# rnissel/Channel-Estimation

Measured on AMD Instinct MI355X. Metric: Monte-Carlo channel realisations/sec at 24sc x 14sym; BER curve match vs ref, higher is better.
Workload: dtype f64; 1 GPU; C2: OFDM 24sc x 14sym, N=540, Jakes 500 km/h VehA, 256-QAM, 16 pilots, 7 SNR (10:5:40 dB) x (one-tap + 4 IC) x (MMSE + perfect CSI); engine_batch=65536, parallelism=dp1

## Files before the change

channel-estimation_amd/csrc/dsce_api.hip:

```cpp
#include <math.h>
#include <stdlib.h>
#include <string.h>

#include <algorithm>
#include <functional>
#include <map>
#include <memory>
#include <stdexcept>
#include <string>
#include <cstdio>
#include <thread>
#include <vector>

#include <rccl/rccl.h>
#include <rocprofiler-sdk-roctx/roctx.h>

#include "dsce.h"
#include "dsce_kernels.h"

struct TraceRange {
    explicit TraceRange(const char* m) { roctxRangePushA(m); }
    ~TraceRange() { roctxRangePop(); }
    TraceRange(const TraceRange&) = delete;
    TraceRange& operator=(const TraceRange&) = delete;
// ... 1662 lines not shown
        if (r2 != DSCE_OK) return api_fail(ctx, r2, member_name(ctx, m) + ": " + member(ctx, m)->err);
    }
    return DSCE_OK;
}

template <class F>
static int fanout_par(dsce_ctx* ctx, F&& f) {
    if (!ctx || ctx->peers.empty()) return f(ctx);
    const size_t n = ctx->peers.size() + 1;
    std::vector<int> rc(n, DSCE_OK);
    std::vector<std::thread> th;
    try {
        for (size_t m = 1; m < n; ++m) th.emplace_back([&, m] { rc[m] = f(member(ctx, m)); });
    } catch (const std::exception& e) {
        for (auto& t : th) t.join();
        return api_fail(ctx, DSCE_ENOMEM, std::string("cannot start a member thread: ") + e.what());
    }
    rc[0] = f(ctx);
    for (auto& t : th) t.join();
    if (rc[0] != DSCE_OK) return rc[0];
    for (size_t m = 1; m < n; ++m)
        if (rc[m] != DSCE_OK) return api_fail(ctx, rc[m], member_name(ctx, m) + ": " + member(ctx, m)->err);
    return DSCE_OK;
}

static void shard_slice(uint64_t first, uint64_t n, size_t world, size_t m, uint64_t& f, uint64_t& k) {
    const uint64_t blocks = (n + 63) / 64;
    const uint64_t lo = std::min<uint64_t>(blocks * m / world * 64, n);
    const uint64_t hi = std::min<uint64_t>(blocks * (m + 1) / world * 64, n);
    f = first + lo;
    k = hi - lo;
}

extern "C" {

int dsce_abi_version(void) { return DSCE_ABI_VERSION; }

int dsce_device_count(int* count) {
    int n = 0;
    if (hipGetDeviceCount(&n) != hipSuccess) n = 0;
    if (count) *count = n;
    return DSCE_OK;
}

int dsce_create(int hip_device, dsce_ctx** out) {
    if (!out) return DSCE_EINVAL;
    *out = nullptr;
    auto* ctx = new (std::nothrow) dsce_ctx();
    if (!ctx) return DSCE_ENOMEM;
    ctx->device = hip_device;
    try {
        DSCE_HIP_CHECK(hipSetDevice(hip_device));
        DSCE_HIP_CHECK(hipStreamCreateWithFlags(&ctx->stream, hipStreamNonBlocking));
    } catch (const std::exception& e) {
        delete ctx;
        return DSCE_EHIP;
    }
    *out = ctx;
    return DSCE_OK;
}

int dsce_create_multi(const int32_t* devices, int32_t n_devices, dsce_ctx** out) {
    if (!out) return DSCE_EINVAL;
    *out = nullptr;
    if (!devices || n_devices < 1 || n_devices > 64) {
        fprintf(stderr, "dsce_create_multi: 1..64 devices expected\n");
        return DSCE_EINVAL;
    }
    int count = 0;
    if (hipGetDeviceCount(&count) != hipSuccess) count = 0;
    bool distinct = true;
    for (int i = 0; i < n_devices; ++i) {
        if (devices[i] < 0 || devices[i] >= count) {
            fprintf(stderr, "dsce_create_multi: device %d of %d is not a HIP device\n", (int)devices[i], count);
            return DSCE_EINVAL;
        }
        for (int j = 0; j < i; ++j) distinct = distinct && devices[j] != devices[i];
    }
    dsce_ctx* ctx = nullptr;
    int rc = dsce_create(devices[0], &ctx);
    if (rc != DSCE_OK) return rc;
    for (int i = 1; i < n_devices; ++i) {
        dsce_ctx* p = nullptr;
        rc = dsce_create(devices[i], &p);
        if (rc != DSCE_OK) {
            (void)dsce_destroy(ctx);
            return rc;
        }
        ctx->peers.push_back(p);
    }
    if (distinct) {
        ctx->comms.assign(n_devices, nullptr);
        const ncclResult_t r = ncclCommInitAll(ctx->comms.data(), n_devices, devices);
        if (r != ncclSuccess) {
            fprintf(stderr, "dsce_create_multi: ncclCommInitAll failed: %s\n", ncclGetErrorString(r));
            ctx->comms.clear();
            (void)dsce_destroy(ctx);
            return DSCE_EHIP;
        }
        ctx->reduce = DSCE_REDUCE_RCCL;
    } else {
        ctx->reduce = DSCE_REDUCE_HOST;
    }
    (void)hipSetDevice(devices[0]);
    *out = ctx;
    return DSCE_OK;
// ... 1059 lines not shown
            b += w.bytes;
        }
    }
    if (flops_per_rep) *flops_per_rep = f;
    if (bytes_per_rep) *bytes_per_rep = b;
    API_END
}

int dsce_structured_check(dsce_ctx* ctx, int32_t id, double* out) {
    API_BEGIN
    check_ctx(ctx);
    Scheme& s = get_scheme(ctx, id);
    if (!out) throw ApiError(DSCE_EINVAL, "null output");
    out[0] = s.mic_check;
    out[1] = s.mic_dev;
    out[2] = s.mic_wmax;
    out[3] = s.mic_rtol;
    out[4] = s.lr_resid;
    out[5] = s.Bz ? 1.0 : 0.0;
    out[6] = s.lr_ratio;
    API_END
}

int dsce_fp64_mfma_peak(dsce_ctx* ctx, double* tflops) {
    API_BEGIN
    check_ctx(ctx);
    if (!tflops) throw ApiError(DSCE_EINVAL, "null output");
    int cus = 0;
    DSCE_HIP_CHECK(hipDeviceGetAttribute(&cus, hipDeviceAttributeMultiprocessorCount, ctx->device));
    const int blocks = cus * 8, iters = 4096;
    double* out = dalloc<double>(ctx, (size_t)blocks * 256);
    hipEvent_t e0 = get_event(ctx), e1 = get_event(ctx);
    launch_mfma_f64_peak(ctx->stream, blocks, iters, out);
    float best = 1e30f;
    for (int rep = 0; rep < 3; ++rep) {
        DSCE_HIP_CHECK(hipEventRecord(e0, ctx->stream));
        launch_mfma_f64_peak(ctx->stream, blocks, iters, out);
        DSCE_HIP_CHECK(hipEventRecord(e1, ctx->stream));
        DSCE_HIP_CHECK(hipEventSynchronize(e1));
        float ms = 0.f;
        DSCE_HIP_CHECK(hipEventElapsedTime(&ms, e0, e1));
        best = ms < best ? ms : best;
    }
    DSCE_HIP_CHECK(hipGetLastError());
    ctx->event_pool.push_back(e0);
    ctx->event_pool.push_back(e1);
    free_alloc(ctx, out);
    *tflops = (double)blocks * 4 * iters * PEAK_MFMA_PER_ITER * 2048.0 / (best * 1e-3) / 1e12;
    API_END
}

#define DSCE_OPTIONS(X)                                                                                  \
    X(xcd) X(fuse_stage) X(pic_chain) X(pfuse) X(stage_split) X(noise_fuse) \
    X(snr_chunk) X(jakes_rpw) X(wtrim) X(wcontract_valu) X(mmse_ic) X(jakes_win) X(txrx_fft) X(snr_base) X(jakes_mom) X(realise_win) X(tx_rows) X(mic_lr) X(pic_poly) X(jakes_grp2) X(export_stage_mb)

static int set_option_one(dsce_ctx* ctx, const char* name, int64_t value) {
    API_BEGIN
    check_ctx(ctx);
    if (!name) throw ApiError(DSCE_EINVAL, "null option name");
    const std::string n(name);
    int* slot = nullptr;
#define X(f) if (n == #f) slot = &ctx->op.f;
    DSCE_OPTIONS(X)
#undef X
    if (!slot && (n == "pic_skip" || n == "ic_streams"))
        throw ApiError(DSCE_EINVAL, "option '" + n + "' was retired in r06 (measured neutral in r04 / r05; DESIGN.md 2.0d, 2.0f)");
    if (!slot && (n == "pic_net" || n == "mic_net" || n == "stage_rb" || n == "wrow"))
        throw ApiError(DSCE_EINVAL, "option '" + n + "' was retired: no scheme or channel selected its other values "
                                    "(DESIGN.md 2.0, Pruned after r06)");
    if (!slot) throw ApiError(DSCE_EINVAL, "unknown option '" + n + "'");
    if (n == "jakes_rpw" && value != 1 && value != 2) throw ApiError(DSCE_EINVAL, "jakes_rpw: 1 | 2");
    if (n == "pic_chain" && value != 0 && value != 3)
        throw ApiError(DSCE_EINVAL, "pic_chain: 0 (per-iteration passes) | 3 (k_pic_fft); the r01 chains 1 / 2 "
                                    "(k_pic_chain, k_pic_mfma) were retired in r03");
    if (n == "snr_base" && (value < 0 || value > 255)) throw ApiError(DSCE_EINVAL, "snr_base: 0..255");
    if (n == "snr_base") check_noise_streams(ctx, value, ctx->nsnr, max_noise_slot(ctx));
    if (n == "export_stage_mb" && value < 1) throw ApiError(DSCE_EINVAL, "export_stage_mb: >= 1 (MiB)");
    if (value < -1 || value > 1 << 20) throw ApiError(DSCE_EINVAL, "option value out of range");
    *slot = (int)value;
    API_END
}

int dsce_set_option(dsce_ctx* ctx, const char* name, int64_t value) {
    return fanout(ctx, [&](dsce_ctx* c) { return set_option_one(c, name, value); });
}

int dsce_get_option(dsce_ctx* ctx, const char* name, int64_t* value) {
    API_BEGIN
    if (!ctx || !name || !value) throw ApiError(DSCE_EINVAL, "null argument");
    const std::string n(name);
    const int* slot = nullptr;
#define X(f) if (n == #f) slot = &ctx->op.f;
    DSCE_OPTIONS(X)
#undef X
    if (!slot) throw ApiError(DSCE_EINVAL, "unknown option '" + n + "'");
    *value = *slot;
    API_END
}
#undef DSCE_OPTIONS

int dsce_path_info(dsce_ctx* ctx, int32_t id, uint32_t* flags) {
    API_BEGIN
    check_ctx(ctx);
    Scheme& s = get_scheme(ctx, id);
    if (!flags) throw ApiError(DSCE_EINVAL, "null output");
    *flags = s.path;
    API_END
}

int dsce_jakes_info(dsce_ctx* ctx, int32_t* out6) {
    API_BEGIN
    check_ctx(ctx);
    if (!out6) throw ApiError(DSCE_EINVAL, "null output");
    const JakesInfo& ji = ctx->jakes_info;
    out6[0] = ji.kernel;
    out6[1] = ji.grp2;
    out6[2] = ji.ngrp;
    out6[3] = ji.lg;
    out6[4] = ji.mt;
    out6[5] = ji.nchunk;
    API_END
}

int dsce_scheme_dims(dsce_ctx* ctx, int32_t id, dsce_dims* dims) {
    API_BEGIN
    if (!ctx) throw ApiError(DSCE_EINVAL, "null context");
    Scheme& s = get_scheme(ctx, id);
    if (!dims) throw ApiError(DSCE_EINVAL, "null output");
    dims->n_samples = s.N;
// ... 14 lines not shown
```

channel-estimation_amd/csrc/dsce_kernels.h:

```cpp
#pragma once

#include "dsce_common.h"

#include <vector>

namespace dsce {

struct Opts {
    int xcd = 1;
    int fuse_stage = 1;
    int pic_chain = 3;
    int pfuse = 1;
    int stage_split = 0;
    int noise_fuse = 1;
    int snr_chunk = 0;
    int jakes_rpw = 2;
    int wtrim = 1;
    int wcontract_valu = 0;
    int mmse_ic = 1;
    int jakes_win = 1;
    int txrx_fft = 1;
    int snr_base = 0;
    int tx_rows = 1;
    int realise_win = 0;
    int mic_lr = 1;
    int pic_poly = 1;
    int jakes_grp2 = 1;
    int jakes_mom = 2;
    int export_stage_mb = 1024;
};

enum : unsigned {
    PATH_WPAIR3_FUSED = 1u << 0,
    PATH_WPAIR3 = 1u << 1,
    PATH_WPAIR4M = 1u << 2,
    PATH_WCONTRACT_VALU = 1u << 3,
    PATH_PIC_MFMA = 1u << 4,
    PATH_PIC_CHAIN = 1u << 5,
    PATH_PIC_PASSES = 1u << 6,
    PATH_STAGE_FUSED = 1u << 7,
    PATH_STAGE_SPLIT = 1u << 8,
    PATH_NOISE_FUSED = 1u << 9,
    PATH_PIC_FFT = 1u << 10,
    PATH_MIC_FFT = 1u << 11,
    PATH_TXRX_FFT = 1u << 12,
    PATH_PILOT_FUSED = 1u << 13,
    PATH_MIC_STAGES = 1u << 14,
    PATH_MIC_LR = 1u << 15,
    PATH_PIC_POLY = 1u << 16,
    PATH_WROW3 = 1u << 17,
};

struct TraceK {
    int unit;
    int LK, ND;
    double2* yest;
    double2* yperf;
    double2* hest;
    int* dec_e;
    int* dec_p;
    int U;
};
__device__ __forceinline__ bool trace_hit(const TraceK* t, int unit) { return t->U > 0 || unit == t->unit; }
__device__ __forceinline__ size_t trace_ix(const TraceK* t, size_t e, int unit) {
    return t->U > 0 ? e * (size_t)t->U + (size_t)unit : e;
}
template <bool BULK>
__device__ __forceinline__ bool trace_hit(const TraceK* t, int unit) {
    if constexpr (BULK) return true;
    else return unit == t->unit;
}
template <bool BULK>
__device__ __forceinline__ size_t trace_ix(const TraceK* t, size_t e, int unit) {
    if constexpr (BULK) return e * (size_t)t->U + (size_t)unit;
    else return e;
}

struct McBuffers {
    int R;
    int rvalid;
    int nsnr;
    int U;
    int snr0;
    double2* ir;
    double2* xp;
    uint16_t* sidx;
    double2* r0;
    double2* h;
    double2* xs;
    double2* ss;
    double2* y;
    double2* yest;
    double2* yperf;
    double2* hp;
    double2* hp2;
    double2* hest;
    double2* v;
    double2* u;
    double2* t;
    double2* e;
    double2* e2;
    uint16_t* qe;
    uint16_t* qp;
// ... 162 lines not shown
```

channel-estimation_amd/csrc/kernels_mc.hip:

```cpp
#include "dsce_kernels.h"
#include "bm_tables.h"

#include <math.h>
#include <algorithm>
#include <stdexcept>
#include <type_traits>
#include <stdlib.h>
#include <string.h>

namespace dsce {

static constexpr double TWO_PI = 6.283185307179586;
static constexpr int WAVE = 64;

__device__ __forceinline__ int wave_sum(int v) {
#pragma unroll
    for (int o = 32; o > 0; o >>= 1) v += __shfl_xor(v, o, 64);
    return v;
}
__device__ __forceinline__ int wave_sum_dpp(int v) {
    v += __builtin_amdgcn_update_dpp(0, v, 0xb1, 0xf, 0xf, false);
    v += __builtin_amdgcn_update_dpp(0, v, 0x4e, 0xf, 0xf, false);
    v += __builtin_amdgcn_update_dpp(0, v, 0x141, 0xf, 0xf, false);
    v += __builtin_amdgcn_update_dpp(0, v, 0x140, 0xf, 0xf, false);
// ... 1401 lines not shown
    {0.25881904510252076, 0.96592582628906829},
    {0.0, 1.0},
    {-0.25881904510252076, 0.96592582628906829},
    {-0.5, 0.86602540378443865},
    {-0.70710678118654752, 0.70710678118654752},
    {-0.86602540378443865, 0.5},
    {-0.96592582628906829, 0.25881904510252076}};

template <int S>
__device__ __forceinline__ void dft3(double2& a, double2& b, double2& c) {
    constexpr double H = 0.86602540378443865;
    const double2 t = c_add(b, c), d = c_sub(b, c);
    const double2 m = make_double2(fma(-0.5, t.x, a.x), fma(-0.5, t.y, a.y));
    a = c_add(a, t);
    b = make_double2(fma(-S * H, d.y, m.x), fma(S * H, d.x, m.y));
    c = make_double2(fma(S * H, d.y, m.x), fma(-S * H, d.x, m.y));
}

__device__ __forceinline__ double2 c_mulf(double2 a, double2 b) {
    return make_double2(fma(a.x, b.x, -(a.y * b.y)), fma(a.x, b.y, a.y * b.x));
}


__device__ __forceinline__ double2 mfma4_cmul(double2 a, double2 b) {
    double re = __builtin_amdgcn_mfma_f64_4x4x4f64(a.x, b.x, 0.0, 0, 0, 0);
    re = __builtin_amdgcn_mfma_f64_4x4x4f64(a.y, b.y, re, 0, 0, 1);
    double im = __builtin_amdgcn_mfma_f64_4x4x4f64(a.x, b.y, 0.0, 0, 0, 0);
    im = __builtin_amdgcn_mfma_f64_4x4x4f64(a.y, b.x, im, 0, 0, 0);
    return make_double2(re, im);
}

__device__ __forceinline__ double2 bperm_c(int addr, double2 v) {
    return make_double2(__hiloint2double(__builtin_amdgcn_ds_bpermute(addr, __double2hiint(v.x)),
                                         __builtin_amdgcn_ds_bpermute(addr, __double2loint(v.x))),
                        __hiloint2double(__builtin_amdgcn_ds_bpermute(addr, __double2hiint(v.y)),
                                         __builtin_amdgcn_ds_bpermute(addr, __double2loint(v.y))));
}

__host__ __device__ constexpr int p6(int k) { return (6 - k) % 6; }

template <int S>
__device__ __forceinline__ void dft6(double2 (&x)[6]) {
    dft3<S>(x[0], x[2], x[4]);
    dft3<S>(x[3], x[5], x[1]);
#pragma unroll
    for (int k2 = 0; k2 < 3; ++k2) {
        const int i0 = 2 * k2, i1 = (2 * k2 + 3) % 6;
        const double2 a = x[i0], b = x[i1];
        x[i0] = c_add(a, b);
        x[i1] = c_sub(a, b);
    }
}

template <int NT, int SH, bool TRACE, bool S0>
__device__ __forceinline__ void pic_fft_body(const SchemeK& sk, const BandOrder& ord, const double2* __restrict__ ir, int N,
                                             const StorePerfectDetect& o, int niter, int vb, int vn) {
    int ug, blk;
    band_block(ord, sk.QH.nblk, ug, blk, vb, vn);
    const int tid = threadIdx.x, l = tid & 63, w = tid >> 6, r = l >> 4;
    const int U = o.U, R = o.R;
    const int unit = ug * WAVE + w * 16 + (l & 15);
    const int rl = unit % R;
    const int row0 = sk.QH.row0[blk], klo = sk.QH.klo[blk];
    const double cs = o.scI, rq = o.rQ;
    __shared__ double2 sym[256];
    __shared__ unsigned sgridw[64];
    const unsigned char* sgrid = (const unsigned char*)sgridw;
    __shared__ double2 rpv[24];
    __shared__ int rdc[24];
    __shared__ double2 amt[2][6][16];
    __shared__ int cntl[4][PM_MAXIT + 1];
    __shared__ double2 ucst[6][256];
    double2 u[6], yh[6], hc[6];
    unsigned txp[2] = {0u, 0u};
    double2 taps[6][NT];
    const __amdgpu_buffer_rsrc_t trs =
        buf_rsrc(ir + (size_t)klo * R, ((size_t)(NT - 1) * N + (N - klo)) * R * sizeof(double2));
    const unsigned tv0 = (unsigned)(6 * r * R + rl) * 16u;
    {
        const double2 a = sk.ct_symc[tid];
        const unsigned gw = sk.ct_grid[min(tid, 63)];
        const int rt = min(tid, 23);
        const double2 pv = sk.ct_rpv[blk * 24 + rt];
        const int rdv = sk.ct_rdc[blk * 24 + rt];
        const double2 nt = sk.ct_amt[min(tid, 191)];
        const RowView vu = S0 ? RowView(o.xs, row0, R, r, rl, 16) : RowView(o.u, row0, U, r, unit, 16);
        const RowView vs(o.sidr, row0, R, r, rl, 2), vy(o.y, row0, U, r, unit, 16), vh(o.h, row0, R, r, rl, 16);
#pragma unroll
        for (int b = 0; b < 6; ++b) {
            u[b] = vu.ld2(b);
            txp[b >> 2] |= (vs.ldu16(b) & 0xffu) << (8 * (b & 3));
            yh[b] = vy.ld2(b);
            hc[b] = vh.ld2(b);
        }
#pragma unroll
        for (int m = 0; m < 6; ++m)
#pragma unroll
            for (int q = 0; q < NT; ++q) taps[m][q] = buf_ld2(trs, tv0, (unsigned)((q * N + m) * R) * 16u);
        sym[tid] = a;
        sgridw[min(tid, 63)] = gw;
        rpv[rt] = pv;
        rdc[rt] = rdv;
        (&amt[0][0][0])[min(tid, 191)] = nt;
    }
    __syncthreads();
#pragma unroll
    for (int q = 0; q < NT; ++q) {
        double2 sq = taps[0][q];
#pragma unroll
        for (int m = 1; m < 6; ++m) sq = c_add(sq, taps[m][q]);
        sq = make_double2(__builtin_amdgcn_mfma_f64_4x4x4f64(1.0, sq.x, 0.0, 0, 0, 0),
                          __builtin_amdgcn_mfma_f64_4x4x4f64(1.0, sq.y, 0.0, 0, 0, 0));
        const double2 mq = make_double2(sq.x * (1.0 / 24.0), sq.y * (1.0 / 24.0));
#pragma unroll
        for (int m = 0; m < 6; ++m) taps[m][q] = c_sub(taps[m][q], mq);
    }
#pragma unroll
    for (int a = 0; a < 6; ++a) {
        u[a] = make_double2(u[a].x * cs, u[a].y * cs);
        ucst[a][tid] = u[a];
    }
    unsigned dmask = 0u, emask = 0u;
#pragma unroll
    for (int a = 0; a < 6; ++a) {
        const int dc = rdc[4 * a + r];
        dmask |= dc >= 0 ? 1u << a : 0u;
        emask |= dc >= 0 && (dc & 1) ? 1u << a : 0u;
    }
    int ncnt = 0;
    auto cweight = [&](int a) -> int {
        return ((dmask >> a) & 1) ? (((emask >> a) & 1) ? 0x10001 : 1) : 0;
    };
    auto reprecode = [&](const int (&dp)[6]) {
        double2 nv[6];
        if (o.pv_uni) {
#pragma unroll
            for (int a = 0; a < 6; ++a) nv[a] = ((dmask >> a) & 1) ? sym[dp[a]] : ucst[a][tid];
        } else {
#pragma unroll
            for (int a = 0; a < 6; ++a) {
                const double2 pr = c_mulf(rpv[4 * a + r], sym[dp[a]]), cv = ucst[a][tid];
                nv[a] = ((dmask >> a) & 1) ? pr : cv;
            }
        }
#pragma unroll
        for (int a = 0; a < 6; ++a) u[a] = nv[a];
    };
    if (S0) {
        int dp[6];
        double fI[6], fQ[6];
#pragma unroll
        for (int a = 0; a < 6; ++a) {
            const double2 hh = hc[a], yv = yh[a];
            const double id = recip_fast(hh.x * hh.x + hh.y * hh.y);
            hc[a] = make_double2(hh.x * id, -hh.y * id);
            const double2 ys = c_mulf(yv, hc[a]);
            yh[a] = make_double2(fma(ys.x, cs, o.ofI), ys.y * cs);
            fI[a] = yh[a].x;
            fQ[a] = fma(yh[a].y, rq, o.ofQ);
        }
        slice6(dp, fI, fQ, o.topI, o.topQ, sgrid);
#pragma unroll
        for (int a = 0; a < 6; ++a) {
            const bool data = (dmask >> a) & 1;
            ncnt += __umul24(__popc((unsigned)(dp[a] ^ (int)((txp[a >> 2] >> (8 * (a & 3))) & 0xffu))), cweight(a));
            if (TRACE && data && trace_hit(o.tr, unit)) o.tr->dec_p[trace_ix(o.tr, (size_t)(rdc[4 * a + r] >> 1), unit)] = dp[a];
        }
        reprecode(dp);
        cntl[w][0] = wave_sum_dpp(rl < o.rvalid ? ncnt : 0);
        ncnt = 0;
    }
    for (int it = 1; it <= niter; ++it) {
        int oz = 0;
        asm volatile("" : "+v"(oz));
        double2 x[6];
#pragma unroll
        for (int a = 0; a < 6; ++a) x[a] = u[a];
        dft6<1>(x);
        double2 t[6];
        const int ai = (l & 3) + 4 * (l >> 4) + oz;
#pragma unroll
        for (int m = 0; m < 6; ++m) {
            const double2 am = amt[0][m][ai], b = x[p6(m)];
            t[m] = mfma4_cmul(am, b);
        }
        const double2 tprev = bperm_c(((l + 48) & 63) * 4, t[5]);
#pragma unroll
        for (int m = 5; m >= 0; --m) {
            const double2 tp = m ? t[m - 1] : tprev;
            double2 acc = make_double2(0.0, 0.0);
#pragma unroll
            for (int q = 0; q < NT; ++q) c_fma(acc, taps[m][q], ((SH >> q) & 1) ? tp : t[m]);
            t[m] = acc;
        }
#pragma unroll
        for (int m = 0; m < 6; ++m) x[m] = mfma4_cmul(amt[1][m][ai], t[m]);
        dft6<-1>(x);
        if (it == 1 && !S0)
#pragma unroll
            for (int a = 0; a < 6; ++a) {
                const double2 hh = hc[a], yv = yh[a];
                const double id = recip_fast(hh.x * hh.x + hh.y * hh.y);
                hc[a] = make_double2(hh.x * id, -hh.y * id);
                const double2 ys = c_mulf(yv, hc[a]);
                yh[a] = make_double2(fma(ys.x, cs, o.ofI), ys.y * cs);
            }
        int dp[6];
        double fI[6], fQ[6];
#pragma unroll
        for (int a = 0; a < 6; ++a) {
            const double2 xa = x[p6(a)], hh = hc[a];
            fI[a] = fma(-xa.x, hh.x, fma(xa.y, hh.y, yh[a].x));
            fQ[a] = fma(fma(-xa.x, hh.y, fma(-xa.y, hh.x, yh[a].y)), rq, o.ofQ);
            if (TRACE && ((dmask >> a) & 1) && o.tr->yperf && trace_hit(o.tr, unit)) {
                const int row = row0 + 4 * a + r;
                const double2 yv = o.y[(size_t)row * U + unit];
                o.tr->yperf[trace_ix(o.tr, (size_t)it * o.tr->LK + row, unit)] = c_sub(yv, make_double2(xa.x / cs, xa.y / cs));
            }
        }
        slice6(dp, fI, fQ, o.topI, o.topQ, sgrid);
#pragma unroll
        for (int a = 0; a < 6; ++a) {
            const bool data = (dmask >> a) & 1;
            ncnt += __umul24(__popc((unsigned)(dp[a] ^ (int)((txp[a >> 2] >> (8 * (a & 3))) & 0xffu))), cweight(a));
            if (TRACE && data && trace_hit(o.tr, unit))
                o.tr->dec_p[trace_ix(o.tr, (size_t)it * o.tr->ND + (rdc[4 * a + r] >> 1), unit)] = dp[a];
        }
        if (it < niter) reprecode(dp);
        cntl[w][it] = wave_sum_dpp(rl < o.rvalid ? ncnt : 0);
        ncnt = 0;
    }
    __syncthreads();
    constexpr int it0 = S0 ? 0 : 1;
    if (tid < 2 * (niter + 1 - it0)) {
        const int it = (tid >> 1) + it0, edge = tid & 1;
        int v = 0;
#pragma unroll
        for (int k = 0; k < 4; ++k) v += (cntl[k][it] >> (16 * edge)) & 0xffff;
        const int snr = o.snr0 + (ug * WAVE) / R;
        const size_t i0 = o.cidx0 + (size_t)it + (size_t)snr * o.cstride_snr + (edge ? (size_t)o.cstride_edge : 0);
        if (v) atomicAdd(&o.counters[i0], (unsigned long long)v);
    }
}

template <int NT, int SH, bool TRACE, bool S0 = false>
__global__ void __launch_bounds__(256) __attribute__((amdgpu_waves_per_eu(2, 2)))
k_pic_fft(SchemeK sk, BandOrder ord, const double2* __restrict__ ir, int N, StorePerfectDetect o, int niter) {
    pic_fft_body<NT, SH, TRACE, S0>(sk, ord, ir, N, o, niter, blockIdx.x, gridDim.x);
}


struct Mic2Args {
    const double2* __restrict__ bv;
    const double2* __restrict__ bs;
    double2* hpa;
    const int* blks;
    int nb;
    double* mse_err;
    double* mse_pow;
    int nsnr, N, nblk, niter, scheme;
    const double2* bz;
    double2* za;
    const double* tw;
    const double* ts;
};

__device__ __forceinline__ int mic_var(int s, int niter) { return (s == 0 || 2 * s <= niter) ? 0 : 1; }

template <int NT, int NP, class ALoad>
__device__ __forceinline__ void mic_taps(double2 (&taps)[6][NT], const ALoad& A, const double2 (&hb)[NP / 4], int l) {
    constexpr int NIDX = 6 * NT, NTILE = (NIDX + 3) / 4, NKS = NP / 4;
    const int g = l >> 4, jc = l & 15, ca = jc & 3, ka = jc >> 2;
    double br[NKS], bi[NKS], bsm[NKS];
#pragma unroll
    for (int ks = 0; ks < NKS; ++ks) {
        br[ks] = hb[ks].x;
        bi[ks] = hb[ks].y;
        bsm[ks] = hb[ks].x + hb[ks].y;
    }
#pragma unroll
    for (int t = 0; t < NTILE; ++t) {
        const int idx = 4 * t + ka;
        const bool ok = (NIDX % 4 == 0) || idx < NIDX;
        const int q = idx >= 6 ? 1 : 0, m = idx - 6 * q;
        d4 p1 = d4{0.0, 0.0, 0.0, 0.0}, p2 = p1, p3 = p1;
#pragma unroll
        for (int ks = 0; ks < NKS; ++ks) {
            const double2 a = A(ok ? q : 0, 6 * ca + (ok ? m : 0), 4 * ks + g);
            const double ar = ok ? a.x : 0.0, ai = ok ? a.y : 0.0;
            p1 = MFMA64(ar, br[ks], p1);
            p2 = MFMA64(ai, bi[ks], p2);
            p3 = MFMA64(ar + ai, bsm[ks], p3);
        }
#pragma unroll
        for (int k = 0; k < 4; ++k) {
            const int id2 = 4 * t + k;
            if (id2 < NIDX) taps[id2 % 6][id2 / 6] = make_double2(p1[k] - p2[k], p3[k] - p1[k] - p2[k]);
        }
    }
}

// ... 785 lines not shown
    ma.niter = niter;
    ma.scheme = pd->scheme;
    ma.bz = mm.Bz;
    ma.za = b.za;
    ma.tw = mm.Tw;
    ma.ts = mm.Ts;
    ma.blks = mm.pblk;
    ma.nb = mm.npb;
    return ma;
}

unsigned launch_mmse_stages(hipStream_t s, const SchemeK& sk, const MmseK& mm, const ChannelK& ch, McBuffers& b,
                            const PerfectDetectArgs* pd, int niter, int xcd, int part, bool lr) {
    StorePerfectDetect o = chain_detect(sk, b, pd, 0);
    Mic2Args ma = mic2_args(sk, mm, ch, b, pd, niter);
    const bool use_lr = lr && mm.Bz && mm.Tw && mm.Ts && b.za && mm.npb == MIC_NB;
    const int sh = pic_fft_shift(ch);
    ma.blks = mm.pblk;
    ma.nb = mm.npb;
    if (part & 1) {
        const dim3 grid(b.U / 16), blk(64 * mm.npb);
#define LAUNCH_MP(NTV, SHV)                                                                                  \
    do {                                                                                                     \
        if (use_lr && b.tr) hipLaunchKernelGGL((k_mic_pilot<NTV, SHV, 16, true, true>), grid, blk, 0, s, sk, ma, o); \
        else if (use_lr) hipLaunchKernelGGL((k_mic_pilot<NTV, SHV, 16, false, true>), grid, blk, 0, s, sk, ma, o); \
        else if (b.tr) hipLaunchKernelGGL((k_mic_pilot<NTV, SHV, 16, true>), grid, blk, 0, s, sk, ma, o);   \
        else hipLaunchKernelGGL((k_mic_pilot<NTV, SHV, 16, false>), grid, blk, 0, s, sk, ma, o);            \
    } while (0)
        if (ch.ntap == 1) LAUNCH_MP(1, 0);
        else if (sh == 1) LAUNCH_MP(2, 1);
        else LAUNCH_MP(2, 2);
#undef LAUNCH_MP
    }
    ma.blks = mm.dblk;
    ma.nb = mm.ndb;
    if (part & 2) {
        const BandOrder om{b.U / WAVE, b.U / b.R, b.R / WAVE, xcd};
        const dim3 grid((b.U / WAVE) * mm.ndb), blk(256);
#define LAUNCH_MD(NTV, SHV)                                                                                  \
    do {                                                                                                     \
        if (use_lr && b.tr) hipLaunchKernelGGL((k_mic_data<NTV, SHV, 16, true, true>), grid, blk, 0, s, sk, om, ma, o); \
        else if (use_lr) hipLaunchKernelGGL((k_mic_data<NTV, SHV, 16, false, true>), grid, blk, 0, s, sk, om, ma, o); \
        else if (b.tr) hipLaunchKernelGGL((k_mic_data<NTV, SHV, 16, true>), grid, blk, 0, s, sk, om, ma, o); \
        else hipLaunchKernelGGL((k_mic_data<NTV, SHV, 16, false>), grid, blk, 0, s, sk, om, ma, o);         \
    } while (0)
        if (ch.ntap == 1) LAUNCH_MD(1, 0);
        else if (sh == 1) LAUNCH_MD(2, 1);
        else LAUNCH_MD(2, 2);
#undef LAUNCH_MD
    }
    return PATH_MIC_FFT | PATH_MIC_STAGES | (use_lr ? PATH_MIC_LR : 0u);
}

unsigned launch_perfect_chain(hipStream_t s, const Opts& op, const SchemeK& sk, const ChannelK& ch, McBuffers& b,
                              const PerfectDetectArgs* pd, int niter, bool stage0) {
    if (!pic_fft_ok(op, sk, ch, b, niter))
        throw std::logic_error("launch_perfect_chain: no chain kernel for this scheme (perfect_chain_ok is false)");
    StorePerfectDetect o = chain_detect(sk, b, pd, 1);
    const BandOrder om{b.U / WAVE, b.U / b.R, b.R / WAVE, op.xcd};
    const dim3 grid((b.U / WAVE) * sk.QH.nblk), blk(256);
    if (!(o.scI != 0.0))
        throw std::logic_error("launch_perfect_chain: the chain's slicer scale is zero");
#define LAUNCH_PF(NTV, SHV, S0V)                                                                               \
    do {                                                                                                        \
        if (b.tr)                                                                                               \
            hipLaunchKernelGGL((k_pic_fft<NTV, SHV, true, S0V>), grid, blk, 0, s, sk, om, b.ir, ch.N, o, niter);  \
        else                                                                                                    \
            hipLaunchKernelGGL((k_pic_fft<NTV, SHV, false, S0V>), grid, blk, 0, s, sk, om, b.ir, ch.N, o, niter); \
    } while (0)
#define LAUNCH_PF2(NTV, SHV)                        \
    do {                                            \
        if (stage0) LAUNCH_PF(NTV, SHV, true);      \
        else LAUNCH_PF(NTV, SHV, false);            \
    } while (0)
    const int sh = pic_fft_shift(ch);
    if (ch.ntap == 1) LAUNCH_PF2(1, 0);
    else if (sh == 1) LAUNCH_PF2(2, 1);
    else LAUNCH_PF2(2, 2);
#undef LAUNCH_PF2
#undef LAUNCH_PF
    return PATH_PIC_FFT;
}

struct PolyArgs {
    const double2* __restrict__ u;
    double2* __restrict__ v;
    double2* __restrict__ fo;
    double2* __restrict__ fo2;
    const double2* __restrict__ C;
    const double2* __restrict__ E;
    const double* __restrict__ A;
    const double* __restrict__ B;
    const double2* __restrict__ tw;
    const double2* __restrict__ ir;
    int U, R, K, N, xcd;
    int delay[4];
};

template <int F, int S>
__device__ __forceinline__ double2 poly_tw(double2 x, int e, const double2* __restrict__ tw) {
    const int i = ((S * e) % F + F) % F;
    if (i == 0) return x;
    return c_mulf(x, tw[i]);
}

template <int F, int S, class Emit>
__device__ __forceinline__ void poly_dft(double2 (&x)[F], const double2* __restrict__ tw, Emit&& emit) {
    static_assert(F % 3 == 0, "F = 3 F2");
    constexpr int F2 = F / 3;
    constexpr double H3 = 0.86602540378443864676;
#pragma unroll
    for (int l2 = 0; l2 < F2; ++l2) {
        const double2 x0 = x[l2], x1 = x[F2 + l2], x2 = x[2 * F2 + l2];
        const double2 sm = c_add(x1, x2), df = c_sub(x1, x2);
        const double2 mm = make_double2(fma(-0.5, sm.x, x0.x), fma(-0.5, sm.y, x0.y));
        const double2 jd = make_double2(-S * H3 * df.y, S * H3 * df.x);
        x[l2] = c_add(x0, sm);
        x[F2 + l2] = poly_tw<F, S>(c_add(mm, jd), l2, tw);
        x[2 * F2 + l2] = poly_tw<F, S>(c_sub(mm, jd), 2 * l2, tw);
    }
#pragma unroll
    for (int m1 = 0; m1 < 3; ++m1)
#pragma unroll
        for (int m2 = 0; m2 < F2; ++m2) {
            double2 acc = x[F2 * m1];
#pragma unroll
            for (int l2 = 1; l2 < F2; ++l2) {
                const int i = ((S * 3 * l2 * m2) % F + F) % F;
                if (i == 0) acc = c_add(acc, x[F2 * m1 + l2]);
                else c_fma(acc, x[F2 * m1 + l2], tw[i]);
            }
            emit(m1 + 3 * m2, acc);
        }
}
// ... 948 lines not shown
```

channel-estimation_amd/dsce/engine.py:

```python
from __future__ import annotations

import ctypes as C
import os

import numpy as np

_HERE = os.path.dirname(os.path.abspath(__file__))
LIB_PATH = os.environ.get("DSCE_LIB", os.path.join(_HERE, "libdsce.so"))

EXPORTED = [
    "dsce_abi_version", "dsce_device_count", "dsce_create", "dsce_destroy", "dsce_last_error",
    "dsce_set_channel", "dsce_set_snr", "dsce_add_scheme", "dsce_build_mmse", "dsce_set_batch", "dsce_run",
    "dsce_bits_per_rep", "dsce_channel_realise", "dsce_get_correlation", "dsce_get_W", "dsce_trace_unit",
    "dsce_enable_timing", "dsce_kernel_time", "dsce_work_model", "dsce_mmse_onetap", "dsce_tx_matrices",
    "dsce_set_noise_slot", "dsce_set_interpolation", "dsce_enable_mse", "dsce_get_mse", "dsce_trace_unit_ex",
    "dsce_scheme_dims", "dsce_path_info", "dsce_set_option", "dsce_get_option", "dsce_fp64_mfma_peak",
    "dsce_kernel_work", "dsce_structured_check", "dsce_create_multi", "dsce_group_info",
    "dsce_transmission_matrix", "dsce_jakes_info", "dsce_export", "dsce_export_stages",
]

ABI_VERSION = 10

EXPORT_F32 = 1 << 0
EXPORT_DEVICE = 1 << 1
EXPORT_FIELDS = ("y", "hp_ls", "h_est", "h", "xp", "sym")
STAGE_FIELDS = ("hp_ls", "h_est", "y_ic", "dec_est", "dec_perf")
_STAGE_INT = ("dec_est", "dec_perf")

JAKES_KERNELS = {0: "none", 1: "static", 2: "discrete", 3: "full", 4: "win_rec", 5: "win_mom", 6: "win_grp"}

REDUCE = {0: "none", 1: "rccl", 2: "host"}

PATH_BITS = {
    "wpair3_fused": 1 << 0, "wpair3": 1 << 1, "wpair4m": 1 << 2, "wcontract_valu": 1 << 3, "pic_mfma": 1 << 4,
    "pic_chain": 1 << 5, "pic_passes": 1 << 6, "stage_fused": 1 << 7, "stage_split": 1 << 8, "noise_fused": 1 << 9,
    "pic_fft": 1 << 10, "mic_fft": 1 << 11, "txrx_fft": 1 << 12, "pilot_fused": 1 << 13, "mic_stages": 1 << 14,
    "mic_lr": 1 << 15, "pic_poly": 1 << 16, "wrow3": 1 << 17,
}


class ChannelDesc(C.Structure):
    _fields_ = [("n_samples", C.c_int32), ("n_taps", C.c_int32), ("sampling_rate", C.c_double),
                ("max_doppler", C.c_double), ("n_paths", C.c_int32), ("doppler_model", C.c_int32),
                ("pdp_norm", C.POINTER(C.c_double))]


class SchemeDesc(C.Structure):
    _fields_ = [("n_subcarriers", C.c_int32), ("n_symbols", C.c_int32), ("n_tx_symbols", C.c_int32),
                ("n_pilots", C.c_int32), ("n_data", C.c_int32), ("mod_order", C.c_int32),
                ("bits_per_symbol", C.c_int32), ("despread", C.c_int32), ("real_detect", C.c_int32),
                ("bits_slot", C.c_int32), ("pilot_slot", C.c_int32), ("kappa", C.c_double),
                ("data_div", C.c_double), ("G", C.POINTER(C.c_double)), ("Q", C.POINTER(C.c_double)),
                ("P", C.POINTER(C.c_double)), ("pilot_pos", C.POINTER(C.c_int32)),
                ("data_pos", C.POINTER(C.c_int32)), ("considered", C.POINTER(C.c_uint8)),
                ("symbols", C.POINTER(C.c_double))]


class Dims(C.Structure):
    _fields_ = [("n_samples", C.c_int32), ("n_taps", C.c_int32), ("lk", C.c_int32), ("n_pilots", C.c_int32),
                ("n_data", C.c_int32), ("n_tx_symbols", C.c_int32), ("n_schemes", C.c_int32), ("n_snr", C.c_int32),
                ("n_iter", C.c_int32), ("n_counters", C.c_int64)]


class Trace(C.Structure):
    _fields_ = [("y", C.POINTER(C.c_double)), ("h_perfect", C.POINTER(C.c_double)),
                ("hp_stages", C.POINTER(C.c_double)), ("hest_stages", C.POINTER(C.c_double)),
                ("yest_stages", C.POINTER(C.c_double)), ("yperf_stages", C.POINTER(C.c_double)),
                ("dec_est", C.POINTER(C.c_int32)), ("dec_perf", C.POINTER(C.c_int32))]


class ExportOut(C.Structure):
    _fields_ = [("y", C.c_void_p), ("hp_ls", C.c_void_p), ("h_est", C.c_void_p), ("h", C.c_void_p),
                ("xp", C.c_void_p), ("sym", C.POINTER(C.c_int32))]


class ExportStagesOut(C.Structure):
    _fields_ = [("hp_ls", C.c_void_p), ("h_est", C.c_void_p), ("y_ic", C.c_void_p),
                ("dec_est", C.POINTER(C.c_int32)), ("dec_perf", C.POINTER(C.c_int32))]


class TxDesc(C.Structure):
    _fields_ = [("kind", C.c_int32), ("n_subcarriers", C.c_int32), ("n_symbols", C.c_int32),
                ("n_samples", C.c_int32), ("fft_size", C.c_int32), ("intermediate_bin", C.c_int32),
                ("time_spacing", C.c_int32), ("cyclic_prefix", C.c_int32), ("zero_guard", C.c_int32),
                ("proto_len", C.c_int32), ("norm", C.c_double), ("initial_phase", C.c_double),
                ("rx_scale", C.c_double), ("prototype", C.POINTER(C.c_double))]


_lib = None

# ... 458 lines not shown
```

include/dsce.h:

```cpp
#ifndef DSCE_H
#define DSCE_H

#include <stdint.h>

#ifdef __cplusplus
extern "C" {
#endif

#define DSCE_ABI_VERSION 10

#define DSCE_OK 0
#define DSCE_EINVAL -1
#define DSCE_EHIP -2
#define DSCE_ESTATE -3
#define DSCE_ENOMEM -4

#define DSCE_REDUCE_NONE 0
#define DSCE_REDUCE_RCCL 1
#define DSCE_REDUCE_HOST 2

typedef struct dsce_ctx dsce_ctx;

typedef struct {
    int32_t n_samples;
// ... 37 lines not shown
    int32_t intermediate_bin;
    int32_t time_spacing;
    int32_t cyclic_prefix;
    int32_t zero_guard;
    int32_t proto_len;
    double norm;
    double initial_phase;
    double rx_scale;
    const double* prototype;
} dsce_tx_desc;

typedef struct {
    int32_t n_samples;
    int32_t n_taps;
    int32_t lk;
    int32_t n_pilots;
    int32_t n_data;
    int32_t n_tx_symbols;
    int32_t n_schemes;
    int32_t n_snr;
    int32_t n_iter;
    int64_t n_counters;
} dsce_dims;

typedef struct {
    double* y;
    double* h_perfect;
    double* hp_stages;
    double* hest_stages;
    double* yest_stages;
    double* yperf_stages;
    int32_t* dec_est;
    int32_t* dec_perf;
} dsce_trace;

#define DSCE_PATH_WPAIR3_FUSED    (1u << 0)
#define DSCE_PATH_WPAIR3          (1u << 1)
#define DSCE_PATH_WPAIR4M         (1u << 2)
#define DSCE_PATH_WCONTRACT_VALU  (1u << 3)
#define DSCE_PATH_PIC_MFMA        (1u << 4)
#define DSCE_PATH_PIC_CHAIN       (1u << 5)
#define DSCE_PATH_PIC_PASSES      (1u << 6)
#define DSCE_PATH_STAGE_FUSED     (1u << 7)
#define DSCE_PATH_STAGE_SPLIT     (1u << 8)
#define DSCE_PATH_NOISE_FUSED     (1u << 9)
#define DSCE_PATH_PIC_FFT         (1u << 10)
#define DSCE_PATH_MIC_FFT         (1u << 11)
#define DSCE_PATH_TXRX_FFT        (1u << 12)
#define DSCE_PATH_PILOT_FUSED     (1u << 13)
#define DSCE_PATH_MIC_STAGES      (1u << 14)
#define DSCE_PATH_MIC_LR          (1u << 15)
#define DSCE_PATH_PIC_POLY        (1u << 16)
#define DSCE_PATH_WROW3           (1u << 17)

#define DSCE_JAKES_NONE      0
#define DSCE_JAKES_STATIC    1
#define DSCE_JAKES_DISCRETE  2
#define DSCE_JAKES_FULL      3
#define DSCE_JAKES_WIN_REC   4
#define DSCE_JAKES_WIN_MOM   5
#define DSCE_JAKES_WIN_GRP   6

int dsce_abi_version(void);
int dsce_device_count(int* count);

int dsce_create(int hip_device, dsce_ctx** out);
int dsce_destroy(dsce_ctx* ctx);
const char* dsce_last_error(const dsce_ctx* ctx);

int dsce_create_multi(const int32_t* devices, int32_t n_devices, dsce_ctx** out);
int dsce_group_info(dsce_ctx* ctx, int32_t* n_devices, int32_t* devices, int32_t* reduce);

int dsce_set_channel(dsce_ctx* ctx, const dsce_channel_desc* desc);
int dsce_set_snr(dsce_ctx* ctx, const double* pn_time, int32_t n_snr, int32_t n_iter);
int dsce_add_scheme(dsce_ctx* ctx, const dsce_scheme_desc* desc, int32_t* scheme_id);

int dsce_build_mmse(dsce_ctx* ctx, double zero_threshold);

int dsce_set_batch(dsce_ctx* ctx, int32_t reps_per_batch);

int dsce_run(dsce_ctx* ctx, uint64_t seed, uint64_t first_rep, uint64_t n_rep, int64_t* err_counts);

int dsce_bits_per_rep(dsce_ctx* ctx, int32_t scheme_id, int64_t* bits2);

int dsce_mmse_onetap(dsce_ctx* ctx, int32_t scheme_id, int32_t snr_index, int32_t variant, const double* hp_ls,
                     int32_t n_units, double* h_out);

int dsce_tx_matrices(dsce_ctx* ctx, const dsce_tx_desc* desc, double* G_out, double* Q_out);

int dsce_set_noise_slot(dsce_ctx* ctx, int32_t scheme_id, int32_t slot);

int dsce_set_interpolation(dsce_ctx* ctx, int32_t scheme_id, const double* interp);

int dsce_channel_realise(dsce_ctx* ctx, uint64_t seed, uint64_t rep, double* ir_out);
int dsce_transmission_matrix(dsce_ctx* ctx, int32_t scheme_id, uint64_t seed, uint64_t rep, double* d_out);
int dsce_get_correlation(dsce_ctx* ctx, int32_t scheme_id, double* r_hp, double* r_est, double* r_noi);
int dsce_get_W(dsce_ctx* ctx, int32_t scheme_id, int32_t snr_index, int32_t variant, double* w_out);
int dsce_trace_unit(dsce_ctx* ctx, int32_t scheme_id, uint64_t seed, uint64_t rep, int32_t snr_index,
                    double* y, double* hp_stages, double* hest_stages, double* h_perfect);

int dsce_enable_mse(dsce_ctx* ctx, int32_t enable);
int dsce_get_mse(dsce_ctx* ctx, double* err_sum, double* pow_sum);

int dsce_trace_unit_ex(dsce_ctx* ctx, int32_t scheme_id, uint64_t seed, uint64_t rep, int32_t snr_index,
                       const dsce_trace* out);

// ... 45 lines not shown
```

Measured before the change: 9.850 million realisations/s.

## Loop each perfect-CSI PIC FFT block over its realisation's SNR points

```diff
diff --git a/channel-estimation_amd/csrc/dsce_api.hip b/channel-estimation_amd/csrc/dsce_api.hip
--- a/channel-estimation_amd/csrc/dsce_api.hip
+++ b/channel-estimation_amd/csrc/dsce_api.hip
@@ -1738,6 +1738,7 @@
     try {
         DSCE_HIP_CHECK(hipSetDevice(hip_device));
         DSCE_HIP_CHECK(hipStreamCreateWithFlags(&ctx->stream, hipStreamNonBlocking));
+        DSCE_HIP_CHECK(hipDeviceGetAttribute(&ctx->op.dev_cus, hipDeviceAttributeMultiprocessorCount, hip_device));
     } catch (const std::exception& e) {
         delete ctx;
         return DSCE_EHIP;
@@ -2903,7 +2904,7 @@
 
 #define DSCE_OPTIONS(X)                                                                                  \
     X(xcd) X(fuse_stage) X(pic_chain) X(pfuse) X(stage_split) X(noise_fuse) \
-    X(snr_chunk) X(jakes_rpw) X(wtrim) X(wcontract_valu) X(mmse_ic) X(jakes_win) X(txrx_fft) X(snr_base) X(jakes_mom) X(realise_win) X(tx_rows) X(mic_lr) X(pic_poly) X(jakes_grp2) X(export_stage_mb)
+    X(snr_chunk) X(jakes_rpw) X(wtrim) X(wcontract_valu) X(mmse_ic) X(jakes_win) X(txrx_fft) X(snr_base) X(jakes_mom) X(realise_win) X(tx_rows) X(mic_lr) X(pic_poly) X(jakes_grp2) X(export_stage_mb) X(snr_loop)
 
 static int set_option_one(dsce_ctx* ctx, const char* name, int64_t value) {
     API_BEGIN
@@ -2926,6 +2927,9 @@
                                     "(k_pic_chain, k_pic_mfma) were retired in r03");
     if (n == "snr_base" && (value < 0 || value > 255)) throw ApiError(DSCE_EINVAL, "snr_base: 0..255");
     if (n == "snr_base") check_noise_streams(ctx, value, ctx->nsnr, max_noise_slot(ctx));
+    if (n == "snr_loop" && (value < -1 || value > 1))
+        throw ApiError(DSCE_EINVAL, "snr_loop: 0 (a block per 64 units) | 1 (a block walks its realisations' SNR points) | "
+                                    "-1 (by grid size)");
     if (n == "export_stage_mb" && value < 1) throw ApiError(DSCE_EINVAL, "export_stage_mb: >= 1 (MiB)");
     if (value < -1 || value > 1 << 20) throw ApiError(DSCE_EINVAL, "option value out of range");
     *slot = (int)value;
diff --git a/channel-estimation_amd/csrc/dsce_kernels.h b/channel-estimation_amd/csrc/dsce_kernels.h
--- a/channel-estimation_amd/csrc/dsce_kernels.h
+++ b/channel-estimation_amd/csrc/dsce_kernels.h
@@ -27,6 +27,8 @@
     int pic_poly = 1;
     int jakes_grp2 = 1;
     int jakes_mom = 2;
+    int snr_loop = -1;
+    int dev_cus = 0;
     int export_stage_mb = 1024;
 };
 
@@ -49,6 +51,7 @@
     PATH_MIC_LR = 1u << 15,
     PATH_PIC_POLY = 1u << 16,
     PATH_WROW3 = 1u << 17,
+    PATH_SNR_LOOP = 1u << 18,
 };
 
 struct TraceK {
diff --git a/channel-estimation_amd/csrc/kernels_mc.hip b/channel-estimation_amd/csrc/kernels_mc.hip
--- a/channel-estimation_amd/csrc/kernels_mc.hip
+++ b/channel-estimation_amd/csrc/kernels_mc.hip
@@ -1477,15 +1477,29 @@
     }
 }
 
-template <int NT, int SH, bool TRACE, bool S0>
+static constexpr int PF_LOOP_CNT = 128;
+template <int NT, int SH, bool TRACE, bool S0, bool LOOP = false>
 __device__ __forceinline__ void pic_fft_body(const SchemeK& sk, const BandOrder& ord, const double2* __restrict__ ir, int N,
                                              const StorePerfectDetect& o, int niter, int vb, int vn) {
+    static_assert(!LOOP || S0, "the SNR loop carries stage 0 (u of the stage kernel is per unit)");
     int ug, blk;
-    band_block(ord, sk.QH.nblk, ug, blk, vb, vn);
+    if constexpr (LOOP) {
+        if (ord.xcd) {
+            const int L = xcd_remap(vb, vn);
+            blk = L % sk.QH.nblk;
+            ug = L / sk.QH.nblk;
+        } else {
+            ug = vb % ord.rgs;
+            blk = vb / ord.rgs;
+        }
+    } else {
+        band_block(ord, sk.QH.nblk, ug, blk, vb, vn);
+    }
     const int tid = threadIdx.x, l = tid & 63, w = tid >> 6, r = l >> 4;
     const int U = o.U, R = o.R;
-    const int unit = ug * WAVE + w * 16 + (l & 15);
-    const int rl = unit % R;
+    const int nk = LOOP ? ord.nchunk : 1;
+    const int unit0 = ug * WAVE + w * 16 + (l & 15);
+    const int rl = LOOP ? unit0 : unit0 % R;
     const int row0 = sk.QH.row0[blk], klo = sk.QH.klo[blk];
     const double cs = o.scI, rq = o.rQ;
     __shared__ double2 sym[256];
@@ -1494,14 +1508,16 @@
     __shared__ double2 rpv[24];
     __shared__ int rdc[24];
     __shared__ double2 amt[2][6][16];
-    __shared__ int cntl[4][PM_MAXIT + 1];
+    __shared__ int cntl[4][LOOP ? PF_LOOP_CNT : PM_MAXIT + 1];
     __shared__ double2 ucst[6][256];
     double2 u[6], yh[6], hc[6];
+    double2 yr[LOOP ? 6 : 1];
     unsigned txp[2] = {0u, 0u};
     double2 taps[6][NT];
     const __amdgpu_buffer_rsrc_t trs =
         buf_rsrc(ir + (size_t)klo * R, ((size_t)(NT - 1) * N + (N - klo)) * R * sizeof(double2));
     const unsigned tv0 = (unsigned)(6 * r * R + rl) * 16u;
+    const RowView vy(o.y, row0, U, r, unit0, 16);
     {
         const double2 a = sk.ct_symc[tid];
         const unsigned gw = sk.ct_grid[min(tid, 63)];
@@ -1509,13 +1525,14 @@
         const double2 pv = sk.ct_rpv[blk * 24 + rt];
         const int rdv = sk.ct_rdc[blk * 24 + rt];
         const double2 nt = sk.ct_amt[min(tid, 191)];
-        const RowView vu = S0 ? RowView(o.xs, row0, R, r, rl, 16) : RowView(o.u, row0, U, r, unit, 16);
-        const RowView vs(o.sidr, row0, R, r, rl, 2), vy(o.y, row0, U, r, unit, 16), vh(o.h, row0, R, r, rl, 16);
+        const RowView vu = S0 ? RowView(o.xs, row0, R, r, rl, 16) : RowView(o.u, row0, U, r, unit0, 16);
+        const RowView vs(o.sidr, row0, R, r, rl, 2), vh(o.h, row0, R, r, rl, 16);
 #pragma unroll
         for (int b = 0; b < 6; ++b) {
             u[b] = vu.ld2(b);
             txp[b >> 2] |= (vs.ldu16(b) & 0xffu) << (8 * (b & 3));
-            yh[b] = vy.ld2(b);
+            if constexpr (LOOP) yr[b] = vy.ld2(b);
+            else yh[b] = vy.ld2(b);
             hc[b] = vh.ld2(b);
         }
 #pragma unroll
@@ -1571,107 +1588,130 @@
 #pragma unroll
         for (int a = 0; a < 6; ++a) u[a] = nv[a];
     };
-    if (S0) {
-        int dp[6];
-        double fI[6], fQ[6];
+    if constexpr (LOOP) {
 #pragma unroll
         for (int a = 0; a < 6; ++a) {
-            const double2 hh = hc[a], yv = yh[a];
+            const double2 hh = hc[a];
             const double id = recip_fast(hh.x * hh.x + hh.y * hh.y);
             hc[a] = make_double2(hh.x * id, -hh.y * id);
-            const double2 ys = c_mulf(yv, hc[a]);
-            yh[a] = make_double2(fma(ys.x, cs, o.ofI), ys.y * cs);
-            fI[a] = yh[a].x;
-            fQ[a] = fma(yh[a].y, rq, o.ofQ);
-        }
-        slice6(dp, fI, fQ, o.topI, o.topQ, sgrid);
-#pragma unroll
-        for (int a = 0; a < 6; ++a) {
-            const bool data = (dmask >> a) & 1;
-            ncnt += __umul24(__popc((unsigned)(dp[a] ^ (int)((txp[a >> 2] >> (8 * (a & 3))) & 0xffu))), cweight(a));
-            if (TRACE && data && trace_hit(o.tr, unit)) o.tr->dec_p[trace_ix(o.tr, (size_t)(rdc[4 * a + r] >> 1), unit)] = dp[a];
-        }
-        reprecode(dp);
-        cntl[w][0] = wave_sum_dpp(rl < o.rvalid ? ncnt : 0);
-        ncnt = 0;
-    }
-    for (int it = 1; it <= niter; ++it) {
-        int oz = 0;
-        asm volatile("" : "+v"(oz));
-        double2 x[6];
-#pragma unroll
-        for (int a = 0; a < 6; ++a) x[a] = u[a];
-        dft6<1>(x);
-        double2 t[6];
-        const int ai = (l & 3) + 4 * (l >> 4) + oz;
-#pragma unroll
-        for (int m = 0; m < 6; ++m) {
-            const double2 am = amt[0][m][ai], b = x[p6(m)];
-            t[m] = mfma4_cmul(am, b);
-        }
-        const double2 tprev = bperm_c(((l + 48) & 63) * 4, t[5]);
-#pragma unroll
-        for (int m = 5; m >= 0; --m) {
-            const double2 tp = m ? t[m - 1] : tprev;
-            double2 acc = make_double2(0.0, 0.0);
-#pragma unroll
-            for (int q = 0; q < NT; ++q) c_fma(acc, taps[m][q], ((SH >> q) & 1) ? tp : t[m]);
-            t[m] = acc;
-        }
-#pragma unroll
-        for (int m = 0; m < 6; ++m) x[m] = mfma4_cmul(amt[1][m][ai], t[m]);
-        dft6<-1>(x);
-        if (it == 1 && !S0)
+        }
+    }
+    auto next_y = [&](int k) {
+        const unsigned ko = (unsigned)(min(k + 1, nk - 1) * R) * 16u;
+#pragma unroll
+        for (int a = 0; a < 6; ++a) yr[LOOP ? a : 0] = buf_ld2(vy.rs, vy.voff, (unsigned)a * vy.step + ko);
+    };
+    for (int k = 0; k < nk; ++k) {
+        const int unit = unit0 + k * R;
+        const int cb = LOOP ? k * (niter + 1) : 0;
+        if (S0) {
+            int dp[6];
+            double fI[6], fQ[6];
 #pragma unroll
             for (int a = 0; a < 6; ++a) {
-                const double2 hh = hc[a], yv = yh[a];
-                const double id = recip_fast(hh.x * hh.x + hh.y * hh.y);
-                hc[a] = make_double2(hh.x * id, -hh.y * id);
+                const double2 yv = LOOP ? yr[a] : yh[a];
+                if constexpr (!LOOP) {
+                    const double2 hh = hc[a];
+                    const double id = recip_fast(hh.x * hh.x + hh.y * hh.y);
+                    hc[a] = make_double2(hh.x * id, -hh.y * id);
+                }
                 const double2 ys = c_mulf(yv, hc[a]);
                 yh[a] = make_double2(fma(ys.x, cs, o.ofI), ys.y * cs);
+                fI[a] = yh[a].x;
+                fQ[a] = fma(yh[a].y, rq, o.ofQ);
             }
-        int dp[6];
-        double fI[6], fQ[6];
-#pragma unroll
-        for (int a = 0; a < 6; ++a) {
-            const double2 xa = x[p6(a)], hh = hc[a];
-            fI[a] = fma(-xa.x, hh.x, fma(xa.y, hh.y, yh[a].x));
-            fQ[a] = fma(fma(-xa.x, hh.y, fma(-xa.y, hh.x, yh[a].y)), rq, o.ofQ);
-            if (TRACE && ((dmask >> a) & 1) && o.tr->yperf && trace_hit(o.tr, unit)) {
-                const int row = row0 + 4 * a + r;
-                const double2 yv = o.y[(size_t)row * U + unit];
-                o.tr->yperf[trace_ix(o.tr, (size_t)it * o.tr->LK + row, unit)] = c_sub(yv, make_double2(xa.x / cs, xa.y / cs));
+            if constexpr (LOOP && !TRACE) next_y(k);
+            slice6(dp, fI, fQ, o.topI, o.topQ, sgrid);
+#pragma unroll
+            for (int a = 0; a < 6; ++a) {
+                const bool data = (dmask >> a) & 1;
+                ncnt += __umul24(__popc((unsigned)(dp[a] ^ (int)((txp[a >> 2] >> (8 * (a & 3))) & 0xffu))), cweight(a));
+                if (TRACE && data && trace_hit(o.tr, unit)) o.tr->dec_p[trace_ix(o.tr, (size_t)(rdc[4 * a + r] >> 1), unit)] = dp[a];
             }
-        }
-        slice6(dp, fI, fQ, o.topI, o.topQ, sgrid);
-#pragma unroll
-        for (int a = 0; a < 6; ++a) {
-            const bool data = (dmask >> a) & 1;
-            ncnt += __umul24(__popc((unsigned)(dp[a] ^ (int)((txp[a >> 2] >> (8 * (a & 3))) & 0xffu))), cweight(a));
-            if (TRACE && data && trace_hit(o.tr, unit))
-                o.tr->dec_p[trace_ix(o.tr, (size_t)it * o.tr->ND + (rdc[4 * a + r] >> 1), unit)] = dp[a];
-        }
-        if (it < niter) reprecode(dp);
-        cntl[w][it] = wave_sum_dpp(rl < o.rvalid ? ncnt : 0);
-        ncnt = 0;
+            reprecode(dp);
+            cntl[w][cb] = wave_sum_dpp(rl < o.rvalid ? ncnt : 0);
+            ncnt = 0;
+        }
+        for (int it = 1; it <= niter; ++it) {
+            int oz = 0;
+            asm volatile("" : "+v"(oz));
+            double2 x[6];
+#pragma unroll
+            for (int a = 0; a < 6; ++a) x[a] = u[a];
+            dft6<1>(x);
+            double2 t[6];
+            const int ai = (l & 3) + 4 * (l >> 4) + oz;
+#pragma unroll
+            for (int m = 0; m < 6; ++m) {
+                const double2 am = amt[0][m][ai], b = x[p6(m)];
+                t[m] = mfma4_cmul(am, b);
+            }
+            const double2 tprev = bperm_c(((l + 48) & 63) * 4, t[5]);
+#pragma unroll
+            for (int m = 5; m >= 0; --m) {
+                const double2 tp = m ? t[m - 1] : tprev;
+                double2 acc = make_double2(0.0, 0.0);
+#pragma unroll
+                for (int q = 0; q < NT; ++q) c_fma(acc, taps[m][q], ((SH >> q) & 1) ? tp : t[m]);
+                t[m] = acc;
+            }
+#pragma unroll
+            for (int m = 0; m < 6; ++m) x[m] = mfma4_cmul(amt[1][m][ai], t[m]);
+            dft6<-1>(x);
+            if (it == 1 && !S0)
+#pragma unroll
+                for (int a = 0; a < 6; ++a) {
+                    const double2 hh = hc[a], yv = yh[a];
+                    const double id = recip_fast(hh.x * hh.x + hh.y * hh.y);
+                    hc[a] = make_double2(hh.x * id, -hh.y * id);
+                    const double2 ys = c_mulf(yv, hc[a]);
+                    yh[a] = make_double2(fma(ys.x, cs, o.ofI), ys.y * cs);
+                }
+            int dp[6];
+            double fI[6], fQ[6];
+#pragma unroll
+            for (int a = 0; a < 6; ++a) {
+                const double2 xa = x[p6(a)], hh = hc[a];
+                fI[a] = fma(-xa.x, hh.x, fma(xa.y, hh.y, yh[a].x));
+                fQ[a] = fma(fma(-xa.x, hh.y, fma(-xa.y, hh.x, yh[a].y)), rq, o.ofQ);
+                if (TRACE && ((dmask >> a) & 1) && o.tr->yperf && trace_hit(o.tr, unit)) {
+                    const int row = row0 + 4 * a + r;
+                    const double2 yv = o.y[(size_t)row * U + unit];
+                    o.tr->yperf[trace_ix(o.tr, (size_t)it * o.tr->LK + row, unit)] = c_sub(yv, make_double2(xa.x / cs, xa.y / cs));
+                }
+            }
+            slice6(dp, fI, fQ, o.topI, o.topQ, sgrid);
+#pragma unroll
+            for (int a = 0; a < 6; ++a) {
+                const bool data = (dmask >> a) & 1;
+                ncnt += __umul24(__popc((unsigned)(dp[a] ^ (int)((txp[a >> 2] >> (8 * (a & 3))) & 0xffu))), cweight(a));
+                if (TRACE && data && trace_hit(o.tr, unit))
+                    o.tr->dec_p[trace_ix(o.tr, (size_t)it * o.tr->ND + (rdc[4 * a + r] >> 1), unit)] = dp[a];
+            }
+            if (it < niter) reprecode(dp);
+            cntl[w][cb + it] = wave_sum_dpp(rl < o.rvalid ? ncnt : 0);
+            ncnt = 0;
+        }
+        if constexpr (LOOP && TRACE) next_y(k);
     }
     __syncthreads();
     constexpr int it0 = S0 ? 0 : 1;
-    if (tid < 2 * (niter + 1 - it0)) {
-        const int it = (tid >> 1) + it0, edge = tid & 1;
+    if (tid < 2 * (nk * (niter + 1) - it0)) {
+        const int ci = (tid >> 1) + it0, edge = tid & 1;
+        const int it = LOOP ? ci % (niter + 1) : ci;
         int v = 0;
 #pragma unroll
-        for (int k = 0; k < 4; ++k) v += (cntl[k][it] >> (16 * edge)) & 0xffff;
-        const int snr = o.snr0 + (ug * WAVE) / R;
+        for (int k = 0; k < 4; ++k) v += (cntl[k][ci] >> (16 * edge)) & 0xffff;
+        const int snr = o.snr0 + (LOOP ? ci / (niter + 1) : (ug * WAVE) / R);
         const size_t i0 = o.cidx0 + (size_t)it + (size_t)snr * o.cstride_snr + (edge ? (size_t)o.cstride_edge : 0);
         if (v) atomicAdd(&o.counters[i0], (unsigned long long)v);
     }
 }
 
-template <int NT, int SH, bool TRACE, bool S0 = false>
+template <int NT, int SH, bool TRACE, bool S0 = false, bool LOOP = false>
 __global__ void __launch_bounds__(256) __attribute__((amdgpu_waves_per_eu(2, 2)))
 k_pic_fft(SchemeK sk, BandOrder ord, const double2* __restrict__ ir, int N, StorePerfectDetect o, int niter) {
-    pic_fft_body<NT, SH, TRACE, S0>(sk, ord, ir, N, o, niter, blockIdx.x, gridDim.x);
+    pic_fft_body<NT, SH, TRACE, S0, LOOP>(sk, ord, ir, N, o, niter, blockIdx.x, gridDim.x);
 }
 
 
@@ -2563,26 +2603,37 @@
     return PATH_MIC_FFT | PATH_MIC_STAGES | (use_lr ? PATH_MIC_LR : 0u);
 }
 
+static constexpr int SNR_LOOP_MIN_ROUNDS = 3;
+static bool snr_loop_fills(const Opts& op, long long blocks) {
+    if (op.dev_cus <= 0) throw std::logic_error("snr_loop: the context's CU count is not set (dsce_create)");
+    return blocks >= (long long)SNR_LOOP_MIN_ROUNDS * 2 * op.dev_cus;
+}
+
 unsigned launch_perfect_chain(hipStream_t s, const Opts& op, const SchemeK& sk, const ChannelK& ch, McBuffers& b,
                               const PerfectDetectArgs* pd, int niter, bool stage0) {
     if (!pic_fft_ok(op, sk, ch, b, niter))
         throw std::logic_error("launch_perfect_chain: no chain kernel for this scheme (perfect_chain_ok is false)");
     StorePerfectDetect o = chain_detect(sk, b, pd, 1);
     const BandOrder om{b.U / WAVE, b.U / b.R, b.R / WAVE, op.xcd};
-    const dim3 grid((b.U / WAVE) * sk.QH.nblk), blk(256);
+    const int nk = b.U / b.R;
+    const bool loop_ok = stage0 && (long long)nk * (niter + 1) <= PF_LOOP_CNT;
+    const bool loop = loop_ok && (op.snr_loop == 1 || (op.snr_loop < 0 && nk > 1 &&
+                                                       snr_loop_fills(op, (long long)(b.R / WAVE) * sk.QH.nblk)));
+    const dim3 grid((loop ? b.R / WAVE : b.U / WAVE) * sk.QH.nblk), blk(256);
     if (!(o.scI != 0.0))
         throw std::logic_error("launch_perfect_chain: the chain's slicer scale is zero");
-#define LAUNCH_PF(NTV, SHV, S0V)                                                                               \
-    do {                                                                                                        \
-        if (b.tr)                                                                                               \
-            hipLaunchKernelGGL((k_pic_fft<NTV, SHV, true, S0V>), grid, blk, 0, s, sk, om, b.ir, ch.N, o, niter);  \
-        else                                                                                                    \
-            hipLaunchKernelGGL((k_pic_fft<NTV, SHV, false, S0V>), grid, blk, 0, s, sk, om, b.ir, ch.N, o, niter); \
+#define LAUNCH_PF(NTV, SHV, S0V, LPV)                                                                               \
+    do {                                                                                                             \
+        if (b.tr)                                                                                                    \
+            hipLaunchKernelGGL((k_pic_fft<NTV, SHV, true, S0V, LPV>), grid, blk, 0, s, sk, om, b.ir, ch.N, o, niter);  \
+        else                                                                                                         \
+            hipLaunchKernelGGL((k_pic_fft<NTV, SHV, false, S0V, LPV>), grid, blk, 0, s, sk, om, b.ir, ch.N, o, niter); \
     } while (0)
-#define LAUNCH_PF2(NTV, SHV)                        \
-    do {                                            \
-        if (stage0) LAUNCH_PF(NTV, SHV, true);      \
-        else LAUNCH_PF(NTV, SHV, false);            \
+#define LAUNCH_PF2(NTV, SHV)                               \
+    do {                                                   \
+        if (loop) LAUNCH_PF(NTV, SHV, true, true);         \
+        else if (stage0) LAUNCH_PF(NTV, SHV, true, false); \
+        else LAUNCH_PF(NTV, SHV, false, false);            \
     } while (0)
     const int sh = pic_fft_shift(ch);
     if (ch.ntap == 1) LAUNCH_PF2(1, 0);
@@ -2590,7 +2641,7 @@
     else LAUNCH_PF2(2, 2);
 #undef LAUNCH_PF2
 #undef LAUNCH_PF
-    return PATH_PIC_FFT;
+    return PATH_PIC_FFT | (loop ? PATH_SNR_LOOP : 0u);
 }
 
 struct PolyArgs {
diff --git a/channel-estimation_amd/dsce/engine.py b/channel-estimation_amd/dsce/engine.py
--- a/channel-estimation_amd/dsce/engine.py
+++ b/channel-estimation_amd/dsce/engine.py
@@ -35,7 +35,7 @@
     "wpair3_fused": 1 << 0, "wpair3": 1 << 1, "wpair4m": 1 << 2, "wcontract_valu": 1 << 3, "pic_mfma": 1 << 4,
     "pic_chain": 1 << 5, "pic_passes": 1 << 6, "stage_fused": 1 << 7, "stage_split": 1 << 8, "noise_fused": 1 << 9,
     "pic_fft": 1 << 10, "mic_fft": 1 << 11, "txrx_fft": 1 << 12, "pilot_fused": 1 << 13, "mic_stages": 1 << 14,
-    "mic_lr": 1 << 15, "pic_poly": 1 << 16, "wrow3": 1 << 17,
+    "mic_lr": 1 << 15, "pic_poly": 1 << 16, "wrow3": 1 << 17, "snr_loop": 1 << 18,
 }
 
 
diff --git a/include/dsce.h b/include/dsce.h
--- a/include/dsce.h
+++ b/include/dsce.h
@@ -113,6 +113,7 @@
 #define DSCE_PATH_MIC_LR          (1u << 15)
 #define DSCE_PATH_PIC_POLY        (1u << 16)
 #define DSCE_PATH_WROW3           (1u << 17)
+#define DSCE_PATH_SNR_LOOP        (1u << 18)
 
 #define DSCE_JAKES_NONE      0
 #define DSCE_JAKES_STATIC    1
```

After: 10.40 million realisations/s (median of 6 runs). +5.6%, better.
